# htcr/sam_road

Measured on NVIDIA H100. Metric: 512x512 ViT-B tiles/sec, higher is better.
Workload: dtype f16 operands / f32 accumulate

## Files before the change

include/samroad_b200.h:

```cpp
#ifndef SAMROAD_B200_H_
#define SAMROAD_B200_H_

#include <stddef.h>
#include <stdint.h>

#ifdef __cplusplus
extern "C" {
#endif

#define SAMROAD_ABI_VERSION 5

typedef struct samroad_ctx* samroad_handle_t;

enum { SAMROAD_F32 = 0, SAMROAD_I64 = 1, SAMROAD_I32 = 2, SAMROAD_U8 = 3, SAMROAD_F64 = 4 };

enum { SAMROAD_TOPO_NORMAL = 0, SAMROAD_TOPO_NO_OFFSET = 1, SAMROAD_TOPO_NO_TRANSFORMER = 2 };

typedef struct SamRoadCfg {
  int32_t patch_size;
  int32_t embed_dim;
  int32_t depth;
  int32_t num_heads;
  int32_t window_size;
  int32_t global_attn_indexes[4];
// ... 178 lines not shown
  int64_t cc;
  int64_t penalty;
  int64_t skipped;
  int64_t scored;
  uint64_t sum_fixed[3];
  double sum;
  int32_t n_sources_gt;
  int32_t n_sources_prop;
  int32_t terminals_gt;
  int32_t terminals_prop;
} SamRoadAplsResult;

int samroad_apls_create(int device, const SamRoadAplsCaps* caps, samroad_apls_t* out);
int samroad_apls_destroy(samroad_apls_t A);
int samroad_apls_upload_graph(samroad_apls_t A, int which, int32_t n_nodes, const double* latlon,
                              const int32_t* row_start, const int32_t* col, const int32_t* weight);
int samroad_apls_candidates(samroad_apls_t A, int which, int32_t n_queries, const double* query_latlon,
                            int32_t* out);
int samroad_apls_one_way(samroad_apls_t A, int gt_role, int32_t n_cp, const int32_t* cp_gt, const int32_t* cp_match,
                         double min_distance_filter, SamRoadAplsResult* out, int32_t* dist_gt, int32_t* dist_prop);

int samroad_stream_write_value32(void* addr, uint32_t value, void* stream);
int samroad_stream_wait_value32(void* addr, uint32_t value, void* stream);

int samroad_timing_enable(samroad_handle_t h, int on);
int samroad_timing_read(samroad_handle_t h, char* buf, size_t cap);

size_t samroad_workspace_bytes(samroad_handle_t h, int B);

uint64_t samroad_launch_count(int reset);

const char* samroad_last_error(void);
int samroad_abi_version(void);


int samroad_op_gemm_f16(const void* A, int lda, const void* W, int ldw, int M, int N, int K,
                        const float* bias, int act, void* out16, int ldo, void* stream);
int samroad_op_gemm_f32(const void* A, int lda, const void* W, int ldw, int M, int N, int K,
                        const float* bias, const float* resid, const float* pos, int pos_rows,
                        float* out32, int ldo, void* stream);
int samroad_op_gemm_ln(const void* A, int lda, const void* W, int ldw, int M, int N, int K,
                       const float* bias, const float* resid, const float* gamma,
                       const float* beta, float eps, int group, int act, void* out16, float* out32,
                       float* out_nchw, int tokens, int ldo, void* stream);
int samroad_op_gemm_ref(const void* A, int lda, const void* W, int ldw, int M, int N, int K,
                        float* out32, int ldo, void* stream);
int samroad_op_layernorm(const float* x, const float* gamma, const float* beta, float eps, int M,
                         int D, void* out16, void* stream);
int samroad_op_attention(const void* qkv16, const float* qkv_bias, const float* rel_h,
                         const float* rel_w, int B, int s, int win, int heads, int head_dim,
                         void* out16, void* stream);

void samroad_debug_force_simt_attention(int on);
void samroad_debug_disable_2cta_gemm(int off);

#ifdef __cplusplus
}
#endif
#endif
```

sam_road_b200/_lib.py:

```python
from __future__ import annotations

import ctypes as C
import weakref
from pathlib import Path

_PKG = Path(__file__).resolve().parent
LIB_PATH = _PKG / "libsamroad_b200.so"

F32, I64, I32, U8, F64 = 0, 1, 2, 3, 4
ABI_VERSION = 5
TOPO_NORMAL, TOPO_NO_OFFSET, TOPO_NO_TRANSFORMER = 0, 1, 2
LOSS_BCE, LOSS_FOCAL = 0, 1
ACT_NONE, ACT_GELU, ACT_RELU = 0, 1, 2


class SamRoadCfg(C.Structure):
    _fields_ = [
        ("patch_size", C.c_int32),
        ("embed_dim", C.c_int32),
        ("depth", C.c_int32),
        ("num_heads", C.c_int32),
        ("window_size", C.c_int32),
        ("global_attn_indexes", C.c_int32 * 4),
        ("use_sam_decoder", C.c_int32),
# ... 92 lines not shown
                                            _vp]),
    "samroad_infer_batch_host_wait": (_i, [_vp, _i]),
    "samroad_prc_create": (_i, [_i, C.POINTER(_vp)]),
    "samroad_prc_destroy": (_i, [_vp]),
    "samroad_prc_reset": (_i, [_vp, _vp]),
    "samroad_prc_update": (_i, [_vp, _vp, C.c_int64, _vp, _i, _vp, C.c_int64, _vp]),
    "samroad_prc_compute": (_i, [_vp, C.POINTER(C.c_int64), C.POINTER(C.c_float), _vp]),
    "samroad_prc_read_curve": (_i, [_vp, _vp, _vp, _vp, _vp, _vp, _vp]),
    "samroad_prc_export_keys": (_i, [_vp, _vp, C.c_int64, C.POINTER(C.c_int64), _vp]),
    "samroad_prc_append_keys": (_i, [_vp, _vp, C.c_int64, _vp]),
    "samroad_val_create": (_i, [_i, C.POINTER(_vp)]),
    "samroad_val_destroy": (_i, [_vp]),
    "samroad_val_reset": (_i, [_vp, _vp]),
    "samroad_val_update": (_i, [_vp, _vp, _vp, _vp, _vp, _vp, _vp, _vp, _vp, _i, _i, _i, _i, _i, _vp, _vp]),
    "samroad_val_read": (_i, [_vp, C.POINTER(C.c_int64), C.POINTER(C.c_float), C.POINTER(C.c_int64), _vp]),
    "samroad_train_workspace_bytes": (_i, [_vp, _targs, C.POINTER(C.c_size_t)]),
    "samroad_train_forward": (_i, [_vp, _targs, _vp, _vp, _i, _vp, _i, _vp, _i, _vp, _i, _vp, _vp, _vp, _vp, _vp,
                                   C.c_size_t, _vp, _vp, _vp]),
    "samroad_train_backward": (_i, [_vp, _targs, _vp, _vp, _vp, _i, _vp, C.c_size_t, _vp, _vp]),
    "samroad_update_tensor_device": (_i, [_vp, C.c_char_p, _vp, C.POINTER(C.c_int64), _i, _vp]),
    "samroad_debug_train_dropout_keep": (_i, [_f, C.c_uint64, _i, _i, C.c_int64, _vp, _vp]),
    "samroad_labels_create": (_i, [_i, C.POINTER(SamRoadLabelCfg), C.POINTER(_vp)]),
    "samroad_labels_destroy": (_i, [_vp]),
    "samroad_labels_upload": (_i, [_vp, _vp, _vp, _vp, C.c_int32, _vp, _vp, _vp, _vp, _vp,
                                   C.POINTER(C.c_int32)]),
    "samroad_labels_batch": (_i, [_vp, _i, C.c_uint64, _vp, _vp, _vp, _vp, _vp, _vp, _vp, _vp,
                                  C.POINTER(C.c_int32), _vp]),
    "samroad_debug_labels_batch_draws": (_i, [_vp, _i, _i, C.c_uint64, _vp, _vp, _vp, _vp, _vp, _vp, _vp, _vp, _vp,
                                              _vp, _vp, C.POINTER(C.c_int32), _vp]),
    "samroad_topo_create": (_i, [_i, C.POINTER(SamRoadTopoCaps), C.POINTER(_vp)]),
    "samroad_topo_destroy": (_i, [_vp]),
    "samroad_topo_upload_graph": (_i, [_vp, _i, C.c_int32, _vp, _vp, _vp, _vp, _vp, _vp]),
    "samroad_topo_run": (_i, [_vp, C.c_int32, _vp, _vp, _d, _d, _d, _d, _vp]),
    "samroad_apls_create": (_i, [_i, C.POINTER(SamRoadAplsCaps), C.POINTER(_vp)]),
    "samroad_apls_destroy": (_i, [_vp]),
    "samroad_apls_upload_graph": (_i, [_vp, _i, C.c_int32, _vp, _vp, _vp, _vp]),
    "samroad_apls_candidates": (_i, [_vp, _i, C.c_int32, _vp, _vp]),
    "samroad_apls_one_way": (_i, [_vp, _i, C.c_int32, _vp, _vp, _d, C.POINTER(SamRoadAplsResult), _vp, _vp]),
    "samroad_stream_write_value32": (_i, [_vp, C.c_uint32, _vp]),
    "samroad_stream_wait_value32": (_i, [_vp, C.c_uint32, _vp]),
    "samroad_timing_enable": (_i, [_vp, _i]),
    "samroad_timing_read": (_i, [_vp, C.c_char_p, C.c_size_t]),
    "samroad_workspace_bytes": (C.c_size_t, [_vp, _i]),
    "samroad_launch_count": (C.c_uint64, [_i]),
    "samroad_last_error": (C.c_char_p, []),
    "samroad_abi_version": (_i, []),
    "samroad_op_gemm_f16": (_i, [_vp, _i, _vp, _i, _i, _i, _i, _vp, _i, _vp, _i, _vp]),
    "samroad_op_gemm_f32": (_i, [_vp, _i, _vp, _i, _i, _i, _i, _vp, _vp, _vp, _i, _vp, _i, _vp]),
    "samroad_op_gemm_ln": (_i, [_vp, _i, _vp, _i, _i, _i, _i, _vp, _vp, _vp, _vp, _f, _i, _i,
                                _vp, _vp, _vp, _i, _i, _vp]),
    "samroad_op_gemm_ref": (_i, [_vp, _i, _vp, _i, _i, _i, _i, _vp, _i, _vp]),
    "samroad_op_layernorm": (_i, [_vp, _vp, _vp, _f, _i, _i, _vp, _vp]),
    "samroad_debug_force_simt_attention": (None, [_i]),
    "samroad_debug_disable_2cta_gemm": (None, [_i]),
    "samroad_op_attention": (_i, [_vp, _vp, _vp, _vp, _i, _i, _i, _i, _i, _vp, _vp]),
}

_lib = None


def load() -> C.CDLL:
    global _lib
    if _lib is not None:
        return _lib
    if not LIB_PATH.exists():
        raise RuntimeError(
            f"{LIB_PATH} is missing: build it with `python -m sam_road_b200.build` "
            "(nvcc, sm_90a). sam_road_b200 has no CPU or PyTorch fallback path.")
    lib = C.CDLL(str(LIB_PATH))
    for name, (res, args) in SIGNATURES.items():
        fn = getattr(lib, name)
        fn.restype = res
        fn.argtypes = args
    _lib = lib
    return lib


def last_error() -> str:
    return load().samroad_last_error().decode("utf-8", "replace")


def check(rc: int, what: str) -> None:
    if rc != 0:
        raise RuntimeError(f"{what} failed (code {rc}): {last_error()}")


def refuse_copy(self):
    raise TypeError(f"{type(self).__name__} owns a native handle and cannot be copied or pickled")


class Handle:

    __getstate__ = refuse_copy

    def __init__(self, create: str, destroy: str, *args):
        lib = load()
        h = C.c_void_p()
        check(getattr(lib, create)(*args, C.byref(h)), create)
        self._as_parameter_ = h.value
        self._finalizer = weakref.finalize(self, getattr(lib, destroy), h.value)

    def close(self) -> None:
        self._as_parameter_ = None
        self._finalizer()


# ... 8 lines not shown
```

sam_road_b200/csrc/attention.cu:

```cuda
#include "attention_mma.cuh"
#include "common.cuh"
#include "ops.h"

#define SRB_TRY_RC(expr) do { int _rc = (expr); if (_rc != 0) return _rc; } while (0)

namespace srb {

constexpr int kAttThreads = 128;
constexpr int kAttChunk = 32;

template <int HD>
__global__ void __launch_bounds__(kAttThreads)
encoder_attention_simt_kernel(const __half* __restrict__ qkv, const float* __restrict__ qkv_bias,
                              const float* __restrict__ rel_h, const float* __restrict__ rel_w,
                              int B, int s, int win, int nwin, int heads, float scale,
                              __half* __restrict__ out) {
  extern __shared__ float smem_att[];
  float* sK = smem_att;
  float* sV = sK + kAttChunk * HD;
  float* sRel = sV + kAttChunk * HD;

  const int D = heads * HD;
  const int ld = 3 * D;
  const int head = blockIdx.y % heads;
// ... 106 lines not shown
        }
        sc[r] = acc;
        m_new = fmaxf(m_new, acc);
      }
      const float alpha = __expf(m_run - m_new);
      l_run *= alpha;
#pragma unroll
      for (int c = 0; c < HD; ++c) o[c] *= alpha;
#pragma unroll
      for (int r = 0; r < kAttChunk; ++r) {
        const float p = __expf(sc[r] - m_new);
        l_run += p;
#pragma unroll
        for (int c = 0; c < HD; ++c) o[c] = fmaf(p, sV[r * HD + c], o[c]);
      }
      m_run = m_new;
    }
  }

  if (q_real) {
    const float inv = 1.0f / l_run;
    __half* op = out + (static_cast<size_t>(b) * s * s + gy * s + gx) * D + head * HD;
#pragma unroll
    for (int c = 0; c < HD; c += 8) {
      uint4 u;
      u.x = pack_half2(o[c + 0] * inv, o[c + 1] * inv);
      u.y = pack_half2(o[c + 2] * inv, o[c + 3] * inv);
      u.z = pack_half2(o[c + 4] * inv, o[c + 5] * inv);
      u.w = pack_half2(o[c + 6] * inv, o[c + 7] * inv);
      *reinterpret_cast<uint4*>(op + c) = u;
    }
  }
}

template <int HD>
static int launch_attention_simt(const __half* qkv, const float* qkv_bias, const float* rel_h,
                                 const float* rel_w, int B, int s, int win, int heads, __half* out,
                                 cudaStream_t st) {
  const int nwin = (s + win - 1) / win;
  const size_t smem = (2 * kAttChunk * HD + kAttThreads * 2 * win) * sizeof(float);
  auto kern = encoder_attention_simt_kernel<HD>;
  SRB_CUDA_OK(cudaFuncSetAttribute(kern, cudaFuncAttributeMaxDynamicSharedMemorySize,
                                   static_cast<int>(smem)));
  dim3 grid((win * win + kAttThreads - 1) / kAttThreads, B * nwin * nwin * heads);
  const float scale = 1.0f / sqrtf(static_cast<float>(HD));
  kern<<<grid, kAttThreads, smem, st>>>(qkv, qkv_bias, rel_h, rel_w, B, s, win, nwin, heads, scale,
                                        out);
  SRB_CUDA_OK(cudaGetLastError());
  note_launch();
  return 0;
}

static bool g_force_simt = false;
void attention_force_simt(int mode) { g_force_simt = (mode & 1) != 0; }

int encoder_attention(const __half* qkv, const float* qkv_bias, const float* rel_h,
                      const float* rel_w, int B, int s, int win, int heads, int hd, __half* out,
                      cudaStream_t st) {
  SRB_REQUIRE(win > 0 && win <= 64 && s > 0 && s <= 64, "attention: win=%d s=%d unsupported", win, s);
  if (B <= 0) return 0;
  if (!g_force_simt) {
    if (hd == 64) return launch_attention_mma<64>(qkv, qkv_bias, rel_h, rel_w, B, s, win, heads, out, st);
    if (hd == 80) return launch_attention_mma<80>(qkv, qkv_bias, rel_h, rel_w, B, s, win, heads, out, st);
  }
  if (hd == 64) return launch_attention_simt<64>(qkv, qkv_bias, rel_h, rel_w, B, s, win, heads, out, st);
  if (hd == 80) return launch_attention_simt<80>(qkv, qkv_bias, rel_h, rel_w, B, s, win, heads, out, st);
  set_last_error("attention: head_dim=%d unsupported (64 or 80)", hd);
  return 2;
}

}
```

sam_road_b200/csrc/attention_mma.cuh:

```cuda
#pragma once

#include "common.cuh"
#include "ops.h"

namespace srb {

constexpr int kAmWarps = 4;
constexpr int kAmKC = 64;

template <int HD>
struct AmLayout {
  static constexpr int kRows = 16 * kAmWarps;
  static constexpr int kPitch = HD + 8;
  static constexpr int kQBytes = kRows * kPitch * 2;
  static constexpr int kStageBytes = 2 * kAmKC * kPitch * 2;
  int winP, lg;
  int nslots, nchunks;
  int relH, relPitch;
  int tabRows;
  int relOffset, padOffset, bytes;
  int kvSlots, uTabOffset, uWarpOffset, uWarpBytes;
  int kvBytes;
  __host__ __device__ int wide_rel_offset() const { return 2 * kQBytes + kvBytes; }
  __host__ __device__ int wide_pad_offset() const { return wide_rel_offset() + 2 * kRows * relPitch * 4; }
// ... 652 lines not shown
  }

  const bool loader = tid < RG * NT;
  const int c8 = tid % NT, lr0 = tid / NT;
  const __half* ksrc = img + D + c8 * 8;
  __half* kdst = reinterpret_cast<__half*>(sKV) + lr0 * P + c8 * 8;
  const uint4* kpad = reinterpret_cast<const uint4*>(sPad) + c8;
  auto load_chunk = [&](int c) {
    if (loader) {
      __half* dk = kdst + (c & 1) * (LY::kStageBytes / 2);
      for (int r = lr0; r < kAmKC; r += RG, dk += RG * P) {
        const int k = c * kAmKC + r, kh = k >> lg, kw = k & (winP - 1);
        __half* dv = dk + kAmKC * P;
        if (kh < win && kw < win) {
          if (kh < s && kw < s) {
            const __half* src = ksrc + (kh * s + kw) * ld;
            cp_async16(smem_u32(dk), src);
            cp_async16(smem_u32(dv), src + D);
          } else {
            *reinterpret_cast<uint4*>(dk) = kpad[0];
            *reinterpret_cast<uint4*>(dv) = kpad[NT];
          }
        } else {
          *reinterpret_cast<uint4*>(dk) = make_uint4(0u, 0u, 0u, 0u);
          *reinterpret_cast<uint4*>(dv) = make_uint4(0u, 0u, 0u, 0u);
        }
      }
    }
    cp_async_commit();
  };
  __syncthreads();
  load_chunk(0);

  const float* const rel[2] = {sRel + rA * RP, sRel + (rA + 16) * RP};
  AmTile<HD> t[2];
  t[0].reset();
  t[1].reset();
  for (int c = 0; c < ly.nchunks; ++c) {
    cp_async_wait_all();
    __syncthreads();
    if (c + 1 < ly.nchunks) load_chunk(c + 1);
    if (!active) continue;
    const __half* sK = reinterpret_cast<const __half*>(sKV + (c & 1) * LY::kStageBytes);
    const int k0 = c * kAmKC;
    am_chunk<HD, 2>(t, qa, sK, sK + kAmKC * P, k0, k0 + kAmKC / 2 < ly.nslots, rel, RP, ly.relH, lg, winP,
                    scale_log2e, lane);
  }
  if (!active) return;
  __half* out0 = out + static_cast<size_t>(b) * s * s * D + head * HD;
#pragma unroll
  for (int m = 0; m < 2; ++m) am_store<HD>(t[m], row0 + rA + m * 16, nreal, rx, s, D, out0, lane);
}

static uint64_t g_am_attr_devs[2] = {0, 0};
static uint64_t g_au_attr_devs[2] = {0, 0};
static uint64_t g_aw_attr_devs[2] = {0, 0};

template <int HD> constexpr int kAuWarps = HD == 64 ? 5 : 4;
constexpr int kAuMaxBytes = (228 * 1024) / 2 - 1024;

template <int HD>
int launch_attention_mma(const __half* qkv, const float* qkv_bias, const float* rel_h, const float* rel_w,
                         int B, int s, int win, int heads, __half* out, cudaStream_t st) {
  using LY = AmLayout<HD>;
  constexpr int NW = kAuWarps<HD>;
  const LY ly(win);
  const int nwin = (s + win - 1) / win;
  const float scale_log2e = 1.4426950408889634f / sqrtf(static_cast<float>(HD));
  const bool resident = win < s && ly.unit_bytes(NW) <= kAuMaxBytes;
  const int w0 = win < s ? win : s;
  const bool wide = win >= s;
  const int qblocks = resident ? 1 : ((w0 * w0 + 15) / 16 + (wide ? 2 : 1) * kAmWarps - 1) / ((wide ? 2 : 1) * kAmWarps);
  const long blocks = static_cast<long>(qblocks) * B * nwin * nwin * heads;
  SRB_REQUIRE(blocks <= 2147483647L, "attention: %ld CTAs exceed the grid limit (B=%d s=%d win=%d heads=%d)",
              blocks, B, s, win, heads);
  const unsigned grid = static_cast<unsigned>(blocks);
  if (resident) {
    auto kern = attention_unit_kernel<HD, NW>;
    if (first_use_on_device(&g_au_attr_devs[HD == 80])) {
      SRB_CUDA_OK(cudaFuncSetAttribute(kern, cudaFuncAttributeMaxDynamicSharedMemorySize, kAuMaxBytes));
    }
    kern<<<grid, NW * 32, ly.unit_bytes(NW), st>>>(qkv, qkv_bias, rel_h, rel_w, s, win, nwin, heads, scale_log2e,
                                                   out);
  } else if (wide) {
    auto kern = attention_wide_kernel<HD>;
    if (first_use_on_device(&g_aw_attr_devs[HD == 80])) {
      SRB_CUDA_OK(cudaFuncSetAttribute(kern, cudaFuncAttributeMaxDynamicSharedMemorySize, LY(64).wide_bytes()));
    }
    kern<<<grid, kAmWarps * 32, ly.wide_bytes(), st>>>(qkv, qkv_bias, rel_h, rel_w, s, win, heads, qblocks,
                                                      scale_log2e, out);
  } else {
    auto kern = attention_mma_kernel<HD>;
    if (first_use_on_device(&g_am_attr_devs[HD == 80])) {
      SRB_CUDA_OK(cudaFuncSetAttribute(kern, cudaFuncAttributeMaxDynamicSharedMemorySize, LY(64).bytes));
    }
    kern<<<grid, kAmWarps * 32, ly.bytes, st>>>(qkv, qkv_bias, rel_h, rel_w, s, win, nwin, heads, qblocks,
                                                scale_log2e, out);
  }
  SRB_CUDA_OK(cudaGetLastError());
  note_launch();
  return 0;
}

}
```

sam_road_b200/csrc/common.cuh:

```cuda
#pragma once

#include <cuda.h>
#include <cuda_fp16.h>
#include <cuda_runtime.h>
#include <stdint.h>

namespace srb {

void set_last_error(const char* fmt, ...);
void note_launch(int n);

#define SRB_CUDA_OK(expr)                                                                  \
  do {                                                                                     \
    cudaError_t _e = (expr);                                                               \
    if (_e != cudaSuccess) {                                                               \
      ::srb::set_last_error("%s:%d: %s -> %s", __FILE__, __LINE__, #expr,                  \
                            cudaGetErrorString(_e));                                       \
      return 1;                                                                            \
    }                                                                                      \
  } while (0)

#define SRB_REQUIRE(cond, ...)                                                             \
  do {                                                                                     \
    if (!(cond)) {                                                                         \
// ... 130 lines not shown
      : "r"(smem_u32(bar)), "r"(parity)
      : "memory");
  return ok != 0;
}
__device__ __forceinline__ void mbar_wait(uint64_t* bar, uint32_t parity) {
  while (!mbar_try_wait(bar, parity)) {
  }
}

__device__ __forceinline__ void tma_prefetch_desc(const CUtensorMap* tm) {
  asm volatile("prefetch.tensormap [%0];" ::"l"(reinterpret_cast<uint64_t>(tm)) : "memory");
}
__device__ __forceinline__ void tma_load_2d(void* smem_dst, const CUtensorMap* tm, uint64_t* bar,
                                            int32_t c0, int32_t c1) {
  asm volatile(
      "cp.async.bulk.tensor.2d.shared::cluster.global.mbarrier::complete_tx::bytes"
      " [%0], [%1, {%3, %4}], [%2];"
      ::"r"(smem_u32(smem_dst)), "l"(reinterpret_cast<uint64_t>(tm)), "r"(smem_u32(bar)),
      "r"(c0), "r"(c1)
      : "memory");
}
__device__ __forceinline__ void tma_store_4d(const CUtensorMap* tm, const void* smem_src, int32_t c0,
                                             int32_t c1, int32_t c2, int32_t c3) {
  asm volatile("cp.async.bulk.tensor.4d.global.shared::cta.bulk_group [%0, {%2, %3, %4, %5}], [%1];"
               ::"l"(reinterpret_cast<uint64_t>(tm)), "r"(smem_u32(smem_src)), "r"(c0), "r"(c1), "r"(c2),
               "r"(c3)
               : "memory");
}
__device__ __forceinline__ void bulk_commit_group() {
  asm volatile("cp.async.bulk.commit_group;" ::: "memory");
}
template <int N>
__device__ __forceinline__ void bulk_wait_group_read() {
  asm volatile("cp.async.bulk.wait_group.read %0;" ::"n"(N) : "memory");
}
template <int N>
__device__ __forceinline__ void bulk_wait_group() {
  asm volatile("cp.async.bulk.wait_group %0;" ::"n"(N) : "memory");
}
__device__ __forceinline__ void tma_load_4d(void* smem_dst, const CUtensorMap* tm, uint64_t* bar,
                                            int32_t c0, int32_t c1, int32_t c2, int32_t c3) {
  asm volatile(
      "cp.async.bulk.tensor.4d.shared::cluster.global.mbarrier::complete_tx::bytes"
      " [%0], [%1, {%3, %4, %5, %6}], [%2];"
      ::"r"(smem_u32(smem_dst)), "l"(reinterpret_cast<uint64_t>(tm)), "r"(smem_u32(bar)),
      "r"(c0), "r"(c1), "r"(c2), "r"(c3)
      : "memory");
}

__device__ __forceinline__ uint64_t wgmma_desc_k128(uint32_t smem_addr) {
  uint64_t d = 0;
  d |= static_cast<uint64_t>((smem_addr >> 4) & 0x3FFFu);
  d |= static_cast<uint64_t>(1) << 16;
  d |= static_cast<uint64_t>(1024u >> 4) << 32;
  d |= static_cast<uint64_t>(1) << 62;
  return d;
}
__device__ __forceinline__ void wgmma_fence() {
  asm volatile("wgmma.fence.sync.aligned;" ::: "memory");
}
__device__ __forceinline__ void wgmma_commit() {
  asm volatile("wgmma.commit_group.sync.aligned;" ::: "memory");
}
template <int N>
__device__ __forceinline__ void wgmma_wait() {
  asm volatile("wgmma.wait_group.sync.aligned %0;" ::"n"(N) : "memory");
}
template <int R>
__device__ __forceinline__ void wgmma_fence_operand(float (&d)[R]) {
#pragma unroll
  for (int i = 0; i < R; ++i) asm volatile("" : "+f"(d[i])::"memory");
}
template <int R>
__device__ __forceinline__ void setmaxnreg_inc() {
  asm volatile("setmaxnreg.inc.sync.aligned.u32 %0;" ::"n"(R));
}
template <int R>
__device__ __forceinline__ void setmaxnreg_dec() {
  asm volatile("setmaxnreg.dec.sync.aligned.u32 %0;" ::"n"(R));
}
__device__ __forceinline__ void named_bar_sync(int id, int threads) {
  asm volatile("bar.sync %0, %1;" ::"r"(id), "r"(threads) : "memory");
}

__device__ __forceinline__ void wgmma_m64n128k16(float (&d)[64], uint64_t desc_a, uint64_t desc_b,
                                             uint32_t accumulate) {
  asm volatile(
      "{\n\t"
      ".reg .pred p;\n\t"
      "setp.ne.b32 p, %66, 0;\n\t"
      "wgmma.mma_async.sync.aligned.m64n128k16.f32.f16.f16 "
      "{"
      "%0, %1, %2, %3, %4, %5, %6, %7, %8, %9, %10, %11, %12, %13, %14, %15, "
      "%16, %17, %18, %19, %20, %21, %22, %23, %24, %25, %26, %27, %28, %29, %30, %31, "
      "%32, %33, %34, %35, %36, %37, %38, %39, %40, %41, %42, %43, %44, %45, %46, %47, "
      "%48, %49, %50, %51, %52, %53, %54, %55, %56, %57, %58, %59, %60, %61, %62, %63"
      "}, %64, %65, p, 1, 1, 0, 0;\n\t"
      "}\n"
      : "+f"(d[0]), "+f"(d[1]), "+f"(d[2]), "+f"(d[3]), "+f"(d[4]), "+f"(d[5]), "+f"(d[6]), "+f"(d[7]),
        "+f"(d[8]), "+f"(d[9]), "+f"(d[10]), "+f"(d[11]), "+f"(d[12]), "+f"(d[13]), "+f"(d[14]), "+f"(d[15]),
        "+f"(d[16]), "+f"(d[17]), "+f"(d[18]), "+f"(d[19]), "+f"(d[20]), "+f"(d[21]), "+f"(d[22]), "+f"(d[23]),
        "+f"(d[24]), "+f"(d[25]), "+f"(d[26]), "+f"(d[27]), "+f"(d[28]), "+f"(d[29]), "+f"(d[30]), "+f"(d[31]),
        "+f"(d[32]), "+f"(d[33]), "+f"(d[34]), "+f"(d[35]), "+f"(d[36]), "+f"(d[37]), "+f"(d[38]), "+f"(d[39]),
        "+f"(d[40]), "+f"(d[41]), "+f"(d[42]), "+f"(d[43]), "+f"(d[44]), "+f"(d[45]), "+f"(d[46]), "+f"(d[47]),
        "+f"(d[48]), "+f"(d[49]), "+f"(d[50]), "+f"(d[51]), "+f"(d[52]), "+f"(d[53]), "+f"(d[54]), "+f"(d[55]),
        "+f"(d[56]), "+f"(d[57]), "+f"(d[58]), "+f"(d[59]), "+f"(d[60]), "+f"(d[61]), "+f"(d[62]), "+f"(d[63])
      : "l"(desc_a), "l"(desc_b), "r"(accumulate));
}

__device__ __forceinline__ void wgmma_m64n256k16(float (&d)[128], uint64_t desc_a, uint64_t desc_b,
                                             uint32_t accumulate) {
  asm volatile(
      "{\n\t"
      ".reg .pred p;\n\t"
      "setp.ne.b32 p, %130, 0;\n\t"
      "wgmma.mma_async.sync.aligned.m64n256k16.f32.f16.f16 "
      "{"
      "%0, %1, %2, %3, %4, %5, %6, %7, %8, %9, %10, %11, %12, %13, %14, %15, "
      "%16, %17, %18, %19, %20, %21, %22, %23, %24, %25, %26, %27, %28, %29, %30, %31, "
      "%32, %33, %34, %35, %36, %37, %38, %39, %40, %41, %42, %43, %44, %45, %46, %47, "
      "%48, %49, %50, %51, %52, %53, %54, %55, %56, %57, %58, %59, %60, %61, %62, %63, "
      "%64, %65, %66, %67, %68, %69, %70, %71, %72, %73, %74, %75, %76, %77, %78, %79, "
      "%80, %81, %82, %83, %84, %85, %86, %87, %88, %89, %90, %91, %92, %93, %94, %95, "
      "%96, %97, %98, %99, %100, %101, %102, %103, %104, %105, %106, %107, %108, %109, %110, %111, "
      "%112, %113, %114, %115, %116, %117, %118, %119, %120, %121, %122, %123, %124, %125, %126, %127"
      "}, %128, %129, p, 1, 1, 0, 0;\n\t"
      "}\n"
      : "+f"(d[0]), "+f"(d[1]), "+f"(d[2]), "+f"(d[3]), "+f"(d[4]), "+f"(d[5]), "+f"(d[6]), "+f"(d[7]),
        "+f"(d[8]), "+f"(d[9]), "+f"(d[10]), "+f"(d[11]), "+f"(d[12]), "+f"(d[13]), "+f"(d[14]), "+f"(d[15]),
        "+f"(d[16]), "+f"(d[17]), "+f"(d[18]), "+f"(d[19]), "+f"(d[20]), "+f"(d[21]), "+f"(d[22]), "+f"(d[23]),
        "+f"(d[24]), "+f"(d[25]), "+f"(d[26]), "+f"(d[27]), "+f"(d[28]), "+f"(d[29]), "+f"(d[30]), "+f"(d[31]),
        "+f"(d[32]), "+f"(d[33]), "+f"(d[34]), "+f"(d[35]), "+f"(d[36]), "+f"(d[37]), "+f"(d[38]), "+f"(d[39]),
        "+f"(d[40]), "+f"(d[41]), "+f"(d[42]), "+f"(d[43]), "+f"(d[44]), "+f"(d[45]), "+f"(d[46]), "+f"(d[47]),
        "+f"(d[48]), "+f"(d[49]), "+f"(d[50]), "+f"(d[51]), "+f"(d[52]), "+f"(d[53]), "+f"(d[54]), "+f"(d[55]),
        "+f"(d[56]), "+f"(d[57]), "+f"(d[58]), "+f"(d[59]), "+f"(d[60]), "+f"(d[61]), "+f"(d[62]), "+f"(d[63]),
        "+f"(d[64]), "+f"(d[65]), "+f"(d[66]), "+f"(d[67]), "+f"(d[68]), "+f"(d[69]), "+f"(d[70]), "+f"(d[71]),
        "+f"(d[72]), "+f"(d[73]), "+f"(d[74]), "+f"(d[75]), "+f"(d[76]), "+f"(d[77]), "+f"(d[78]), "+f"(d[79]),
        "+f"(d[80]), "+f"(d[81]), "+f"(d[82]), "+f"(d[83]), "+f"(d[84]), "+f"(d[85]), "+f"(d[86]), "+f"(d[87]),
        "+f"(d[88]), "+f"(d[89]), "+f"(d[90]), "+f"(d[91]), "+f"(d[92]), "+f"(d[93]), "+f"(d[94]), "+f"(d[95]),
        "+f"(d[96]), "+f"(d[97]), "+f"(d[98]), "+f"(d[99]), "+f"(d[100]), "+f"(d[101]), "+f"(d[102]), "+f"(d[103]),
        "+f"(d[104]), "+f"(d[105]), "+f"(d[106]), "+f"(d[107]), "+f"(d[108]), "+f"(d[109]), "+f"(d[110]), "+f"(d[111]),
        "+f"(d[112]), "+f"(d[113]), "+f"(d[114]), "+f"(d[115]), "+f"(d[116]), "+f"(d[117]), "+f"(d[118]), "+f"(d[119]),
        "+f"(d[120]), "+f"(d[121]), "+f"(d[122]), "+f"(d[123]), "+f"(d[124]), "+f"(d[125]), "+f"(d[126]), "+f"(d[127])
      : "l"(desc_a), "l"(desc_b), "r"(accumulate));
}


int make_tmap_f16_2d(CUtensorMap* out, const void* base, uint64_t rows, uint64_t cols,
                     uint64_t ld_elems, uint32_t box_rows, uint32_t box_cols = 64);

int make_tmap_f16_4d(CUtensorMap* out, const void* base, const uint64_t dims[4],
                     const uint64_t strides_elems[3], const uint32_t box[4]);
int make_tmap_f32_4d_dense(CUtensorMap* out, const void* base, const uint64_t dims[4],
                           const uint64_t strides_bytes[3], const uint32_t box[4]);

}
```

sam_road_b200/csrc/model.cu:

```cuda
#include "../../include/samroad_b200.h"

#include <cuda_fp16.h>
#include <cuda_runtime.h>

#include <cstdarg>
#include <cstdio>
#include <cstring>
#include <map>
#include <string>
#include <vector>

#include "common.cuh"
#include "ops.h"

using namespace srb;

namespace {

struct HostTensor {
  std::vector<int64_t> shape;
  std::vector<float> data;
  int64_t numel() const {
    int64_t n = 1;
    for (auto d : shape) n *= d;
// ... 1022 lines not shown
                                         pairs_dtype, valid_host, N, Ns, Np, mask_scores_host,
                                         image_embeddings_host, topo_scores_host));
  return samroad_infer_batch_host_wait(h, 0);
}

extern "C" int samroad_stream_write_value32(void* addr, uint32_t value, void* stream) {
  return stream_write_value32(addr, value, static_cast<cudaStream_t>(stream));
}
extern "C" int samroad_stream_wait_value32(void* addr, uint32_t value, void* stream) {
  return stream_wait_value32_geq(addr, value, static_cast<cudaStream_t>(stream));
}
extern "C" uint64_t samroad_launch_count(int reset) { return launch_count(reset != 0); }
extern "C" const char* samroad_last_error(void) { return get_last_error(); }
extern "C" int samroad_abi_version(void) { return SAMROAD_ABI_VERSION; }

extern "C" int samroad_op_gemm_f16(const void* A, int lda, const void* W, int ldw, int M, int N,
                                   int K, const float* bias, int act, void* out16, int ldo,
                                   void* stream) {
  return gemm_f16out(static_cast<const __half*>(A), lda, static_cast<const __half*>(W), ldw, M, N, K,
                     bias, act, static_cast<__half*>(out16), ldo, static_cast<cudaStream_t>(stream));
}
extern "C" int samroad_op_gemm_f32(const void* A, int lda, const void* W, int ldw, int M, int N,
                                   int K, const float* bias, const float* resid, const float* pos,
                                   int pos_rows, float* out32, int ldo, void* stream) {
  return gemm_f32out(static_cast<const __half*>(A), lda, static_cast<const __half*>(W), ldw, M, N, K,
                     bias, resid, pos, pos_rows, out32, ldo, static_cast<cudaStream_t>(stream));
}
extern "C" int samroad_op_gemm_ln(const void* A, int lda, const void* W, int ldw, int M, int N,
                                  int K, const float* bias, const float* resid, const float* gamma,
                                  const float* beta, float eps, int group, int act, void* out16,
                                  float* out32, float* out_nchw, int tokens, int ldo, void* stream) {
  return gemm_ln(static_cast<const __half*>(A), lda, static_cast<const __half*>(W), ldw, M, N, K,
                 bias, resid, gamma, beta, eps, group, act, static_cast<__half*>(out16), out32,
                 out_nchw, tokens, ldo, static_cast<cudaStream_t>(stream));
}
extern "C" int samroad_op_gemm_ref(const void* A, int lda, const void* W, int ldw, int M, int N,
                                   int K, float* out32, int ldo, void* stream) {
  return gemm_ref_simt(static_cast<const __half*>(A), lda, static_cast<const __half*>(W), ldw, M, N,
                       K, out32, ldo, static_cast<cudaStream_t>(stream));
}
extern "C" int samroad_op_layernorm(const float* x, const float* gamma, const float* beta,
                                    float eps, int M, int D, void* out16, void* stream) {
  return layernorm_f16(x, gamma, beta, eps, M, D, static_cast<__half*>(out16), false,
                       static_cast<cudaStream_t>(stream));
}
extern "C" int samroad_op_attention(const void* qkv16, const float* qkv_bias, const float* rel_h,
                                    const float* rel_w, int B, int s, int win, int heads,
                                    int head_dim, void* out16, void* stream) {
  return encoder_attention(static_cast<const __half*>(qkv16), qkv_bias, rel_h, rel_w, B, s,
                           win, heads, head_dim, static_cast<__half*>(out16),
                           static_cast<cudaStream_t>(stream));
}
extern "C" void samroad_debug_force_simt_attention(int on) { attention_force_simt(on); }
extern "C" void samroad_debug_disable_2cta_gemm(int off) { g_ln_ascending = (off & 16) != 0; }
```

sam_road_b200/csrc/ops.h:

```cpp
#pragma once

#include <cuda_fp16.h>
#include <cuda_runtime.h>
#include <stdint.h>

namespace srb {

enum Act : int { ACT_NONE = 0, ACT_GELU = 1, ACT_RELU = 2 };

void set_last_error(const char* fmt, ...);
const char* get_last_error();
int device_sm_count();
bool first_use_on_device(uint64_t* device_mask);
void note_launch(int n = 1);
int stream_write_value32(void* addr, uint32_t value, cudaStream_t st);
int stream_wait_value32_geq(void* addr, uint32_t value, cudaStream_t st);
uint64_t launch_count(bool reset);

int gemm_f16out(const __half* A, int lda, const __half* W, int ldw, int M, int N, int K,
                const float* bias, int act, __half* out, int ldo, cudaStream_t st);
int gemm_f32out(const __half* A, int lda, const __half* W, int ldw, int M, int N, int K,
                const float* bias, const float* resid, const float* pos, int pos_rows, float* out,
                int ldo, cudaStream_t st);
int gemm_ln(const __half* A, int lda, const __half* W, int ldw, int M, int N, int K,
            const float* bias, const float* resid, const float* gamma, const float* beta, float eps,
            int group, int act, __half* out16, float* out32, float* out_nchw, int tokens, int ldo,
            cudaStream_t st, int conv_s = 0);
int gemm_dec_final(const __half* A, int lda, const __half* W, int ldw, int M, int K,
                   const float* bias3, const float* w4, const float* bias4, int s, int P,
                   float* scores, float* logits, cudaStream_t st);
int gemm_ref_simt(const __half* A, int lda, const __half* W, int ldw, int M, int N, int K,
                  float* out, int ldo, cudaStream_t st);

int layernorm_f16(const float* x, const float* gamma, const float* beta, float eps, int M, int D,
                  __half* out, bool reverse, cudaStream_t st);
int im2col_patch16(const void* rgb, int dtype, int B, int P, const float* mean, const float* inv_std,
                   __half* out, cudaStream_t st);
int crop_tiles(const uint8_t* scene, int H, int W, const int* tile_xy, int B, int P, uint8_t* out,
               cudaStream_t st);
int im2col_3x3(const __half* x, int B, int s, int C, __half* out, cudaStream_t st);
int convert_f32_f16(const float* x, long n, __half* out, cudaStream_t st);

int encoder_attention(const __half* qkv, const float* qkv_bias, const float* rel_h,
                      const float* rel_w, int B, int s, int win, int heads, int hd, __half* out,
                      cudaStream_t st);
void attention_force_simt(int mode);

int topo_sample_features(const float* feat_nchw, int B, int C, int s, int P, const void* points,
                         int pts_dtype, int N, __half* out, cudaStream_t st);
int topo_sample_features_f32(const float* feat_nchw, int B, int C, int s, int P, const void* points,
                             int pts_dtype, int N, float* out, cudaStream_t st);
struct TopoPairInputs {
  const float* pst;
  const float* w_off;
  const float* bias;
  const void* points;
  const void* pairs;
  int pts_dtype, pairs_dtype, N, tokens_per_b, zero_offset;
};
int topo_pair_features(const TopoPairInputs& in, int tokens, float* x32, __half* x16, cudaStream_t st);
int topo_fix_valid(const uint8_t* valid, int rows, int Np, uint8_t* out, cudaStream_t st);
int topo_attention(const __half* qkv, const uint8_t* valid, int rows, int Np, __half* out,
                   cudaStream_t st);
int topo_output(const float* x32, const uint8_t* valid_fixed, const float* w, const float* b,
                int tokens, float* logits, float* scores, cudaStream_t st);

struct TopoLayerParams {
  const float* in_b;
  const float* out_b;
  const float* l1_b;
  const float* l2_b;
  const float *n1_g, *n1_b, *n2_g, *n2_b;
};
int topo_transformer_fused(const TopoPairInputs& in, const __half* w_chunks, const TopoLayerParams* layers,
                           const float* out_w, const float* out_b, const uint8_t* valid_fixed, int tokens,
                           int Np, float* logits, float* scores, cudaStream_t st);

struct SamAttnW { const float *qw, *qb, *kw, *kb, *vw, *vb, *ow, *ob; };
struct SamDecoderWeights {
  const float* tokens;
  const float* q0;
  const float* no_mask_embed;
  const float* dense_pe;
  SamAttnW self_attn[2], t2i[2], i2t[2], final_attn;
  const float *n1g[2], *n1b[2], *n2g[2], *n2b[2], *n3g[2], *n3b[2], *n4g[2], *n4b[2];
  const float *l1w[2], *l1b[2], *l2w[2], *l2b[2];
  const float *nfg, *nfb;
  const float* hw[2][3];
  const float* hb[2][3];
  const __half *t2i_kw16[3], *t2i_vw16[3];
  const __half *i2t_qw16[2], *i2t_ow16[2];
  const __half *up1_w, *up2_w;
  const float *up1_b, *up1_g, *up1_beta, *up2_b;
};
size_t sam_decoder_ws_bytes(int B, int T);
int sam_decoder_prepare(const SamDecoderWeights& w, float* q0_out, cudaStream_t st);
int sam_decoder_forward(const SamDecoderWeights& w, const float* emb_nchw, int B, int s, int P, void* ws,
                        float* mask_scores, float* mask_logits, cudaStream_t st);

// ... 5 lines not shown
```

Before: 1547.

## Add TMA+wgmma warp-specialized kernel for global-attention layers

Adds a dedicated kernel for the global (win == s) attention layers with HD=64. A producer warpgroup TMA-loads K/V chunks into a two-stage mbarrier ring, and two consumer warpgroups run wgmma for QK^T and register-sourced PV with online softmax and decomposed relative-position bias. The consumers alternate issue turns through named barriers. It replaces the earlier mma.sync path for those layers to raise tensor-core throughput on large key counts. The cost is more complexity, a large smem footprint, one CTA per SM and new descriptor-layout assumptions.

```diff
diff --git a/include/samroad_b200.h b/include/samroad_b200.h
--- a/include/samroad_b200.h
+++ b/include/samroad_b200.h
@@ -254,6 +254,7 @@
                          void* out16, void* stream);
 
 void samroad_debug_force_simt_attention(int on);
+int64_t samroad_debug_attention_wgmma_launches(void);
 void samroad_debug_disable_2cta_gemm(int off);
 
 #ifdef __cplusplus
diff --git a/sam_road_b200/_lib.py b/sam_road_b200/_lib.py
--- a/sam_road_b200/_lib.py
+++ b/sam_road_b200/_lib.py
@@ -168,6 +168,7 @@
     "samroad_op_gemm_ref": (_i, [_vp, _i, _vp, _i, _i, _i, _i, _vp, _i, _vp]),
     "samroad_op_layernorm": (_i, [_vp, _vp, _vp, _f, _i, _i, _vp, _vp]),
     "samroad_debug_force_simt_attention": (None, [_i]),
+    "samroad_debug_attention_wgmma_launches": (C.c_int64, []),
     "samroad_debug_disable_2cta_gemm": (None, [_i]),
     "samroad_op_attention": (_i, [_vp, _vp, _vp, _vp, _i, _i, _i, _i, _i, _vp, _vp]),
 }
diff --git a/sam_road_b200/csrc/attention.cu b/sam_road_b200/csrc/attention.cu
--- a/sam_road_b200/csrc/attention.cu
+++ b/sam_road_b200/csrc/attention.cu
@@ -182,7 +182,11 @@
 }
 
 static bool g_force_simt = false;
-void attention_force_simt(int mode) { g_force_simt = (mode & 1) != 0; }
+void attention_force_simt(int mode) {
+  g_force_simt = (mode & 1) != 0;
+  g_ag_small_grids = (mode & 2) != 0;
+}
+long long attention_wgmma_launches() { return g_ag_launches; }
 
 int encoder_attention(const __half* qkv, const float* qkv_bias, const float* rel_h,
                       const float* rel_w, int B, int s, int win, int heads, int hd, __half* out,
diff --git a/sam_road_b200/csrc/attention_mma.cuh b/sam_road_b200/csrc/attention_mma.cuh
--- a/sam_road_b200/csrc/attention_mma.cuh
+++ b/sam_road_b200/csrc/attention_mma.cuh
@@ -728,9 +728,254 @@
   for (int m = 0; m < 2; ++m) am_store<HD>(t[m], row0 + rA + m * 16, nreal, rx, s, D, out0, lane);
 }
 
+constexpr int kAgKC = 128;
+constexpr int kAgStages = 2;
+constexpr int kAgThreads = 384;
+
+struct AgLayout {
+  static constexpr int kQBytes = 128 * 64 * 2;
+  static constexpr int kStageBytes = 2 * kAgKC * 64 * 2;
+  static constexpr int kRingOffset = kQBytes;
+  static constexpr int kTabOffset = kRingOffset + kAgStages * kStageBytes;
+  int winP, lg, nchunks, relH, relPitch, tabRows;
+  int relOffset, barOffset, bytes;
+  __host__ __device__ explicit AgLayout(int win) {
+    winP = 8; lg = 3;
+    while (winP < win) { winP <<= 1; ++lg; }
+    nchunks = (win * winP + kAgKC - 1) / kAgKC;
+    relH = ((nchunks * kAgKC / winP + 7) / 8) * 8;
+    relPitch = ((relH + winP + 31) / 32) * 32 + 4;
+    tabRows = ((2 * win - 1 + 7) / 8) * 8;
+    relOffset = kTabOffset + 4 * tabRows * AmLayout<64>::kPitch * 2;
+    barOffset = relOffset + 128 * relPitch * 4;
+    bytes = barOffset + 64 + 1024;
+  }
+};
+
+__global__ void __launch_bounds__(kAgThreads, 1)
+attention_global_wgmma_kernel(const __grid_constant__ CUtensorMap tmQ, const __grid_constant__ CUtensorMap tmKV,
+                              const float* __restrict__ rel_h, const float* __restrict__ rel_w, int s, int heads,
+                              int qblocks, float scale_log2e, __half* __restrict__ out) {
+  using LY = AgLayout;
+  const LY ly(s);
+  const int win = s, winP = ly.winP, lg = ly.lg, RP = ly.relPitch, relH = ly.relH;
+  extern __shared__ uint8_t smem_ag_raw[];
+  uint8_t* smem = smem_ag_raw + ((1024u - (smem_u32(smem_ag_raw) & 1023u)) & 1023u);
+  __half* sTab = reinterpret_cast<__half*>(smem + LY::kTabOffset);
+  float* sRel = reinterpret_cast<float*>(smem + ly.relOffset);
+  uint64_t* full_bar = reinterpret_cast<uint64_t*>(smem + ly.barOffset);
+  uint64_t* empty_bar = full_bar + kAgStages;
+  uint64_t* q_bar = empty_bar + kAgStages;
+
+  const int D = heads * 64;
+  const int unit = blockIdx.x / qblocks;
+  const int head = unit % heads, b = unit / heads;
+  const int nreal = s * s;
+  const int row0 = (blockIdx.x - unit * qblocks) * 128;
+  const int warp = threadIdx.x >> 5, lane = threadIdx.x & 31;
+
+  if (threadIdx.x == 0) {
+    tma_prefetch_desc(&tmQ);
+    tma_prefetch_desc(&tmKV);
+    for (int st = 0; st < kAgStages; ++st) {
+      mbar_init(&full_bar[st], 1);
+      mbar_init(&empty_bar[st], 8);
+    }
+    mbar_init(q_bar, 1);
+    fence_barrier_init();
+  }
+  __syncthreads();
+
+  if (warp < 4) {
+    setmaxnreg_dec<40>();
+    if (threadIdx.x == 0) {
+      mbar_arrive_expect_tx(q_bar, LY::kQBytes);
+      tma_load_2d(smem, &tmQ, q_bar, head * 64, b * nreal + row0);
+      tma_load_2d(smem + LY::kQBytes / 2, &tmQ, q_bar, head * 64, b * nreal + row0 + 64);
+      const int khc = kAgKC >> lg;
+      for (int c = 0; c < ly.nchunks; ++c) {
+        const int st = c % kAgStages;
+        mbar_wait(&empty_bar[st], ((c / kAgStages) & 1) ^ 1u);
+        uint8_t* sk = smem + LY::kRingOffset + st * LY::kStageBytes;
+        mbar_arrive_expect_tx(&full_bar[st], LY::kStageBytes);
+        tma_load_4d(sk, &tmKV, &full_bar[st], D + head * 64, 0, c * khc, b);
+        tma_load_4d(sk + LY::kStageBytes / 2, &tmKV, &full_bar[st], 2 * D + head * 64, 0, c * khc, b);
+      }
+    }
+    return;
+  }
+
+  setmaxnreg_inc<232>();
+  const int ctid = threadIdx.x - 128;
+  const int g = ctid >> 7, w = (ctid >> 5) & 3;
+  const int rl = 64 * g + 16 * w + (lane >> 2);
+  const int cq = 2 * (lane & 3);
+
+  am_stage_tables<64, 256>(sTab, rel_h, rel_w, win, ly.tabRows, ctid);
+  if (lane < 16) {
+    float* r = sRel + (64 * g + 16 * w + lane) * RP;
+    for (int c = win; c < relH; ++c) r[c] = -INFINITY;
+    for (int c = win; c < winP; ++c) r[relH + c] = -INFINITY;
+  }
+  named_bar_sync(1, 256);
+
+  mbar_wait(q_bar, 0);
+  const uint8_t* sQg = smem + g * (LY::kQBytes / 2);
+  {
+    uint32_t qa[4][4];
+    const int r = 16 * w + (lane & 15);
+#pragma unroll
+    for (int k = 0; k < 4; ++k)
+      ldsm_x4(smem_u32(sQg + r * 128 + (((2 * k + (lane >> 4)) ^ (r & 7)) << 4)), qa[k][0], qa[k][1], qa[k][2],
+              qa[k][3]);
+    am_relpos<64>(qa, sTab, ly.tabRows, win, s, min(row0 + rl, nreal - 1), min(row0 + rl + 8, nreal - 1),
+                  sRel + rl * RP, RP, relH, lane);
+  }
+  __syncwarp();
+  const float* relA = sRel + rl * RP;
+  const float* relB = relA + 8 * RP;
+  float rwA[16][2], rwB[16][2];
+#pragma unroll
+  for (int n = 0; n < 16; ++n)
+#pragma unroll
+    for (int e = 0; e < 2; ++e) {
+      const int kw = (8 * n + cq + e) & (winP - 1);
+      rwA[n][e] = relA[relH + kw];
+      rwB[n][e] = relB[relH + kw];
+    }
+
+  const uint64_t qdesc = wgmma_desc_k128(smem_u32(sQg));
+  float o[32];
+#pragma unroll
+  for (int i = 0; i < 32; ++i) o[i] = 0.f;
+  float mA = -INFINITY, mB = -INFINITY, lA = 0.f, lB = 0.f;
+  const auto turn_begin = [&] { named_bar_sync(2 + g, 256); };
+  const auto turn_end = [&](bool last) {
+    if (!(last && g == 1)) asm volatile("bar.arrive %0, 256;" ::"r"(3 - g) : "memory");
+  };
+  if (g == 1) asm volatile("bar.arrive 2, 256;" ::: "memory");
+  for (int c = 0; c < ly.nchunks; ++c) {
+    const int st = c % kAgStages;
+    mbar_wait(&full_bar[st], (c / kAgStages) & 1);
+    const uint32_t k_addr = smem_u32(smem + LY::kRingOffset + st * LY::kStageBytes);
+    const uint32_t v_addr = k_addr + LY::kStageBytes / 2;
+    float sc[64];
+    const uint64_t kdesc = wgmma_desc_k128(k_addr);
+    turn_begin();
+    wgmma_fence();
+#pragma unroll
+    for (int k = 0; k < 4; ++k)
+      wgmma_m64n128k16(sc, qdesc + static_cast<uint64_t>(2 * k), kdesc + static_cast<uint64_t>(2 * k),
+                       k != 0 ? 1u : 0u);
+    wgmma_commit();
+    turn_end(false);
+    wgmma_wait<0>();
+    wgmma_fence_operand(sc);
+
+    const int k0 = c * kAgKC;
+    float cmA = -INFINITY, cmB = -INFINITY;
+#pragma unroll
+    for (int n = 0; n < 16; ++n) {
+      const int kh = (k0 + 8 * n) >> lg;
+      const float hA = relA[kh], hB = relB[kh];
+      sc[4 * n + 0] = fmaf(sc[4 * n + 0], scale_log2e, hA + rwA[n][0]);
+      sc[4 * n + 1] = fmaf(sc[4 * n + 1], scale_log2e, hA + rwA[n][1]);
+      sc[4 * n + 2] = fmaf(sc[4 * n + 2], scale_log2e, hB + rwB[n][0]);
+      sc[4 * n + 3] = fmaf(sc[4 * n + 3], scale_log2e, hB + rwB[n][1]);
+      cmA = fmaxf(cmA, fmaxf(sc[4 * n + 0], sc[4 * n + 1]));
+      cmB = fmaxf(cmB, fmaxf(sc[4 * n + 2], sc[4 * n + 3]));
+    }
+#pragma unroll
+    for (int off = 1; off <= 2; off <<= 1) {
+      cmA = fmaxf(cmA, __shfl_xor_sync(0xffffffffu, cmA, off));
+      cmB = fmaxf(cmB, __shfl_xor_sync(0xffffffffu, cmB, off));
+    }
+    const float nmA = fmaxf(mA, cmA), nmB = fmaxf(mB, cmB);
+    const float alA = ex2_approx(mA - nmA), alB = ex2_approx(mB - nmB);
+    mA = nmA; mB = nmB;
+    lA *= alA; lB *= alB;
+#pragma unroll
+    for (int j = 0; j < 8; ++j) {
+      o[4 * j + 0] *= alA; o[4 * j + 1] *= alA; o[4 * j + 2] *= alB; o[4 * j + 3] *= alB;
+    }
+    uint32_t pa[8][4];
+#pragma unroll
+    for (int kc = 0; kc < 8; ++kc) {
+#pragma unroll
+      for (int h = 0; h < 2; ++h) {
+        const float* sn = sc + 4 * (2 * kc + h);
+        pa[kc][2 * h + 0] = pack_half2(ex2_approx(sn[0] - mA), ex2_approx(sn[1] - mA));
+        pa[kc][2 * h + 1] = pack_half2(ex2_approx(sn[2] - mB), ex2_approx(sn[3] - mB));
+        const float2 fA = __half22float2(*reinterpret_cast<const __half2*>(&pa[kc][2 * h + 0]));
+        const float2 fB = __half22float2(*reinterpret_cast<const __half2*>(&pa[kc][2 * h + 1]));
+        lA += fA.x + fA.y;
+        lB += fB.x + fB.y;
+      }
+    }
+    wgmma_fence_operand(o);
+    turn_begin();
+    wgmma_fence();
+#pragma unroll
+    for (int kc = 0; kc < 8; ++kc)
+      wgmma_m64n64k16_rs_tb(o, pa[kc], wgmma_desc_mn128(v_addr + kc * 16 * 128), 1u);
+    wgmma_commit();
+    turn_end(c + 1 == ly.nchunks);
+    wgmma_wait<0>();
+    wgmma_fence_operand(o);
+    if (lane == 0) mbar_arrive(&empty_bar[st]);
+  }
+
+#pragma unroll
+  for (int off = 1; off <= 2; off <<= 1) {
+    lA += __shfl_xor_sync(0xffffffffu, lA, off);
+    lB += __shfl_xor_sync(0xffffffffu, lB, off);
+  }
+  const float invA = 1.0f / lA, invB = 1.0f / lB;
+#pragma unroll
+  for (int h = 0; h < 2; ++h) {
+    const int j = row0 + rl + 8 * h;
+    if (j >= nreal) continue;
+    __half* op = out + (static_cast<size_t>(b) * nreal + j) * D + head * 64 + cq;
+    const float inv = h ? invB : invA;
+#pragma unroll
+    for (int j8 = 0; j8 < 8; ++j8)
+      *reinterpret_cast<uint32_t*>(op + j8 * 8) = pack_half2(o[4 * j8 + 2 * h] * inv, o[4 * j8 + 2 * h + 1] * inv);
+  }
+}
+
 static uint64_t g_am_attr_devs[2] = {0, 0};
 static uint64_t g_au_attr_devs[2] = {0, 0};
 static uint64_t g_aw_attr_devs[2] = {0, 0};
+static uint64_t g_ag_attr_devs = 0;
+static bool g_ag_small_grids = false;
+static long long g_ag_launches = 0;
+
+static int launch_attention_global_wgmma(const __half* qkv, const float* rel_h, const float* rel_w, int B, int s,
+                                         int heads, __half* out, cudaStream_t st) {
+  const AgLayout ly(s);
+  const uint64_t D = static_cast<uint64_t>(heads) * 64, ld = 3 * D, n = static_cast<uint64_t>(s);
+  const int qblocks = (s * s + 127) / 128;
+  const long blocks = static_cast<long>(qblocks) * B * heads;
+  SRB_REQUIRE(blocks <= 2147483647L, "attention: %ld CTAs exceed the grid limit (B=%d s=%d heads=%d)", blocks, B, s,
+              heads);
+  CUtensorMap tmQ, tmKV;
+  if (int rc = make_tmap_f16_2d(&tmQ, qkv, static_cast<uint64_t>(B) * n * n, ld, ld, 64)) return rc;
+  const uint64_t dims[4] = {ld, n, n, static_cast<uint64_t>(B)};
+  const uint64_t strides[3] = {ld, n * ld, n * n * ld};
+  const uint32_t box[4] = {64, static_cast<uint32_t>(ly.winP), static_cast<uint32_t>(kAgKC / ly.winP), 1};
+  if (int rc = make_tmap_f16_4d(&tmKV, qkv, dims, strides, box)) return rc;
+  if (first_use_on_device(&g_ag_attr_devs)) {
+    SRB_CUDA_OK(cudaFuncSetAttribute(attention_global_wgmma_kernel, cudaFuncAttributeMaxDynamicSharedMemorySize,
+                                     AgLayout(64).bytes));
+  }
+  const float scale_log2e = 1.4426950408889634f / 8.0f;
+  attention_global_wgmma_kernel<<<static_cast<unsigned>(blocks), kAgThreads, ly.bytes, st>>>(
+      tmQ, tmKV, rel_h, rel_w, s, heads, qblocks, scale_log2e, out);
+  SRB_CUDA_OK(cudaGetLastError());
+  note_launch();
+  ++g_ag_launches;
+  return 0;
+}
 
 template <int HD> constexpr int kAuWarps = HD == 64 ? 5 : 4;
 constexpr int kAuMaxBytes = (228 * 1024) / 2 - 1024;
@@ -738,6 +983,9 @@
 template <int HD>
 int launch_attention_mma(const __half* qkv, const float* qkv_bias, const float* rel_h, const float* rel_w,
                          int B, int s, int win, int heads, __half* out, cudaStream_t st) {
+  if constexpr (HD == 64) {
+    if (win == s && (s > 16 || g_ag_small_grids)) return launch_attention_global_wgmma(qkv, rel_h, rel_w, B, s, heads, out, st);
+  }
   using LY = AmLayout<HD>;
   constexpr int NW = kAuWarps<HD>;
   const LY ly(win);
diff --git a/sam_road_b200/csrc/common.cuh b/sam_road_b200/csrc/common.cuh
--- a/sam_road_b200/csrc/common.cuh
+++ b/sam_road_b200/csrc/common.cuh
@@ -206,6 +206,14 @@
   uint64_t d = 0;
   d |= static_cast<uint64_t>((smem_addr >> 4) & 0x3FFFu);
   d |= static_cast<uint64_t>(1) << 16;
+  d |= static_cast<uint64_t>(1024u >> 4) << 32;
+  d |= static_cast<uint64_t>(1) << 62;
+  return d;
+}
+__device__ __forceinline__ uint64_t wgmma_desc_mn128(uint32_t smem_addr) {
+  uint64_t d = 0;
+  d |= static_cast<uint64_t>((smem_addr >> 4) & 0x3FFFu);
+  d |= static_cast<uint64_t>(1024u >> 4) << 16;
   d |= static_cast<uint64_t>(1024u >> 4) << 32;
   d |= static_cast<uint64_t>(1) << 62;
   return d;
@@ -299,6 +307,24 @@
       : "l"(desc_a), "l"(desc_b), "r"(accumulate));
 }
 
+__device__ __forceinline__ void wgmma_m64n64k16_rs_tb(float (&d)[32], const uint32_t (&a)[4], uint64_t desc_b,
+                                                      uint32_t accumulate) {
+  asm volatile(
+      "{\n\t"
+      ".reg .pred p;\n\t"
+      "setp.ne.b32 p, %37, 0;\n\t"
+      "wgmma.mma_async.sync.aligned.m64n64k16.f32.f16.f16 "
+      "{"
+      "%0, %1, %2, %3, %4, %5, %6, %7, %8, %9, %10, %11, %12, %13, %14, %15, "
+      "%16, %17, %18, %19, %20, %21, %22, %23, %24, %25, %26, %27, %28, %29, %30, %31"
+      "}, {%32, %33, %34, %35}, %36, p, 1, 1, 1;\n\t"
+      "}\n"
+      : "+f"(d[0]), "+f"(d[1]), "+f"(d[2]), "+f"(d[3]), "+f"(d[4]), "+f"(d[5]), "+f"(d[6]), "+f"(d[7]),
+        "+f"(d[8]), "+f"(d[9]), "+f"(d[10]), "+f"(d[11]), "+f"(d[12]), "+f"(d[13]), "+f"(d[14]), "+f"(d[15]),
+        "+f"(d[16]), "+f"(d[17]), "+f"(d[18]), "+f"(d[19]), "+f"(d[20]), "+f"(d[21]), "+f"(d[22]), "+f"(d[23]),
+        "+f"(d[24]), "+f"(d[25]), "+f"(d[26]), "+f"(d[27]), "+f"(d[28]), "+f"(d[29]), "+f"(d[30]), "+f"(d[31])
+      : "r"(a[0]), "r"(a[1]), "r"(a[2]), "r"(a[3]), "l"(desc_b), "r"(accumulate));
+}
 
 int make_tmap_f16_2d(CUtensorMap* out, const void* base, uint64_t rows, uint64_t cols,
                      uint64_t ld_elems, uint32_t box_rows, uint32_t box_cols = 64);
diff --git a/sam_road_b200/csrc/model.cu b/sam_road_b200/csrc/model.cu
--- a/sam_road_b200/csrc/model.cu
+++ b/sam_road_b200/csrc/model.cu
@@ -1098,4 +1098,5 @@
                            static_cast<cudaStream_t>(stream));
 }
 extern "C" void samroad_debug_force_simt_attention(int on) { attention_force_simt(on); }
+extern "C" int64_t samroad_debug_attention_wgmma_launches(void) { return attention_wgmma_launches(); }
 extern "C" void samroad_debug_disable_2cta_gemm(int off) { g_ln_ascending = (off & 16) != 0; }
diff --git a/sam_road_b200/csrc/ops.h b/sam_road_b200/csrc/ops.h
--- a/sam_road_b200/csrc/ops.h
+++ b/sam_road_b200/csrc/ops.h
@@ -45,6 +45,7 @@
                       const float* rel_w, int B, int s, int win, int heads, int hd, __half* out,
                       cudaStream_t st);
 void attention_force_simt(int mode);
+long long attention_wgmma_launches();
 
 int topo_sample_features(const float* feat_nchw, int B, int C, int s, int P, const void* points,
                          int pts_dtype, int N, __half* out, cudaStream_t st);
```

After: 1601, median of 6. 3.5% higher.
